# SamvitJ/Accel

Measured on AMD Instinct MI355X. Metric: frames/sec 1024x2048 Accel-18 kf=5, higher is better.
Workload: dtype f32 (storage, accumulation and results; the launch geometries the tuner picks include the fp32 MFMA, Winograd F(2x2,3x3) and, for most layers, 'fp16x2': each fp32 operand as TWO half terms hi + lo (22-23 significant bits, operands centred in the half range by exact powers of two: weights per channel

## Files before the change

### accel_amd/csrc/accel_hip.cpp

```cpp
#include <hip/hip_runtime.h>
#include <dlfcn.h>
#include <sys/stat.h>
#include <unistd.h>

#include <algorithm>
#include <cmath>
#include <cstdarg>
#include <cstdio>
#include <cstdlib>
#include <cstring>
#include <map>
#include <memory>
#include <sstream>
#include <string>
#include <vector>

#include "../../include/accel_hip.h"
#include "kernels.h"
#include "range.h"

static thread_local std::string g_err;

static int fail(int code, const char* fmt, ...)
{
// ... 479 lines not shown
        c.yH = op.b.H; c.yW = op.b.W;
        if (op.b.H > 2 * op.a.H || op.b.H < 2 * op.a.H - 1 || op.b.W > 2 * op.a.W || op.b.W < 2 * op.a.W - 1)
            return fail(ACCEL_ERR_PLAN, "deconv2x %s: output must be 2x the input (or one row / column less)", op.name.c_str());
    } else {
        int wkh = kh, wkw = kw;
        if (cols) kv_pair(kv, "wk", wkh, wkw, 3, 3);
        if (w->shape[0] != cout || w->shape[1] != cin || w->shape[2] != wkh || w->shape[3] != wkw)
            return fail(ACCEL_ERR_PARAM, "shape inconsistent for %s: need (%d,%d,%d,%d) got (%ld,%ld,%ld,%ld)",
                        wname.c_str(), cout, cin, wkh, wkw, (long)w->shape[0], (long)w->shape[1], (long)w->shape[2], (long)w->shape[3]);
        const int Kreal = wkh * wkw * cin_pad;
        c.K_pad = roundup(Kreal, 32);
        pack_conv_w(*w, cin_pad, rows, c.K_pad, packed);
        if (cols) { c.kh = c.kw = 1; c.Cin = Kreal; }
        else { c.kh = kh; c.kw = kw; c.Cin = cin_pad; }
        c.sh = sh; c.sw = sw; c.ph = ph; c.pw = pw; c.dh = dh; c.dw = dw;
        c.Ho = op.b.H; c.Wo = op.b.W;
        c.yH = op.b.H; c.yW = op.b.W;
        const int eh = (op.a.H + 2 * c.ph - c.dh * (c.kh - 1) - 1) / c.sh + 1;
        const int ew = (op.a.W + 2 * c.pw - c.dw * (c.kw - 1) - 1) / c.sw + 1;
        if (eh != op.b.H || ew != op.b.W)
            return fail(ACCEL_ERR_PLAN, "conv %s: output %dx%d does not match geometry %dx%d", op.name.c_str(), op.b.H, op.b.W, eh, ew);
        if (c.Cin > op.a.Cs) return fail(ACCEL_ERR_PLAN, "conv %s: input view narrower than Cin", op.name.c_str());
    }
    packed.resize(packed.size() + 256, 0.f);
    const char* env_dt = getenv("ACCEL_CONV_DTYPE");
    const int dflt = (p->f16 == 2 || (env_dt && !strcmp(env_dt, "bf16x3"))) ? 2 : (p->f16 || (env_dt && !strcmp(env_dt, "f16"))) ? 1 : 0;
    const int want_f16 = (int)kv_int(kv, "f16", dflt);
    c.f16 = (want_f16 && c.Cin % (want_f16 == 2 ? 4 : 8) == 0 && cout_store > 4) ? want_f16 : 0;
    void* dw_ = nullptr;
    if (c.f16 == 2) {
        std::vector<uint16_t> pb;
        pack_bf16x3(packed, c.deconv2x ? 4 : 1, rows, c.K_pad, pb, c.w_plane);
        if ((rc = dev_upload(p, pb.data(), pb.size() * sizeof(uint16_t), &dw_))) return rc;
    } else if (c.f16) {
        std::vector<_Float16> ph(packed.size());
        for (size_t i = 0; i < packed.size(); ++i) ph[i] = (_Float16)packed[i];
        if ((rc = dev_upload(p, ph.data(), ph.size() * sizeof(_Float16), &dw_))) return rc;
        if (!withheld("b3r")) {
            const int classes = c.deconv2x ? 4 : 1, steps = c.K_pad / 32;
            c.w_plane = (size_t)classes * rows * c.K_pad + 2 * (size_t)rows * 32;
            std::vector<_Float16> pr(c.w_plane, (_Float16)0.f);
            for (int cl = 0; cl < classes; ++cl)
                for (int n = 0; n < rows; ++n)
                    for (int k = 0; k < c.K_pad; ++k)
                        pr[((((size_t)cl * steps + k / 32) * 2 + ((k >> 4) & 1)) * rows + n) * 16 + (k & 15)] = ph[((size_t)cl * rows + n) * c.K_pad + k];
            void* d4 = nullptr;
            if ((rc = dev_upload(p, pr.data(), pr.size() * sizeof(_Float16), &d4))) return rc;
            c.wb3r = d4;
        }
    } else if ((rc = dev_upload(p, packed.data(), packed.size() * sizeof(float), &dw_))) return rc;
    c.w = static_cast<const float*>(dw_);
    {
        const int ft = (int)kv_int(kv, "tile", -1);
        const bool forced = (ft >= CONV_TILE_B3 && ft < CONV_TILE_B3D + CONV_TILE_B3D_N) || (ft >= 90 && ft <= 96);
        if (!c.f16 && c.Cin % 4 == 0 && cout_store > 4 && (!withheld("split") || forced)) {
            std::vector<uint16_t> pb;
            pack_bf16x3(packed, c.deconv2x ? 4 : 1, rows, c.K_pad, pb, c.w_plane);
            void* d3 = nullptr;
            if ((rc = dev_upload(p, pb.data(), pb.size() * sizeof(uint16_t), &d3))) return rc;
            c.wb3 = d3;
            const bool forced_r = (ft >= CONV_TILE_B3R && ft < CONV_TILE_B3D + CONV_TILE_B3D_N) || (ft >= 90 && ft <= 96);
            if (!withheld("b3r") || forced_r) {
                pack_bf16x3r(packed, c.deconv2x ? 4 : 1, rows, c.K_pad, pb, c.w_plane);
                void* d4 = nullptr;
                if ((rc = dev_upload(p, pb.data(), pb.size() * sizeof(uint16_t), &d4))) return rc;
                c.wb3r = d4;
            }
        } else if (forced && !(c.f16 == 1 && c.wb3r && ft >= CONV_TILE_B3R && ft < CONV_TILE_B3D + CONV_TILE_B3D_N)) {
            return fail(ACCEL_ERR_ARG, "conv %s: the bf16x3 kernel takes layers with more than "
                                       "4 output channels only", op.name.c_str());
        }
    }

    std::vector<float> scale(rows, 0.f), shift(rows, 0.f);
    for (int i = 0; i < cout; ++i) scale[i] = 1.f;
    if (kv_has(kv, "bn")) {
        std::vector<float> s, b;
        if ((rc = bn_fold(m, kv_str(kv, "bn"), (float)kv_f(kv, "eps", 1e-5), (int)kv_int(kv, "fixg", 0), cout, s, b))) return rc;
        for (int i = 0; i < cout; ++i) { scale[i] = s[i]; shift[i] = b[i]; }
    }
    if (kv_has(kv, "bias")) {
        const HostParam* bias = get_param(m, kv_str(kv, "bias"));
        if (!bias) return fail(ACCEL_ERR_PARAM, "%s not initialized", kv_str(kv, "bias").c_str());
        if ((int)bias->numel() != cout) return fail(ACCEL_ERR_PARAM, "shape inconsistent for %s", kv_str(kv, "bias").c_str());
        for (int i = 0; i < cout; ++i) shift[i] += bias->data[i] * scale[i];
    }
    if (kv_has(kv, "mul")) {
        const float mul = (float)kv_f(kv, "mul", 1.0);
        for (int i = 0; i < cout; ++i) { scale[i] *= mul; shift[i] *= mul; }
    }
    void *ds = nullptr, *db = nullptr;
    if ((rc = dev_upload(p, scale.data(), rows * sizeof(float), &ds)) ||
        (rc = dev_upload(p, shift.data(), rows * sizeof(float), &db))) return rc;
    c.scale = static_cast<const float*>(ds);
    c.shift = static_cast<const float*>(db);
    {
        const char* sp = getenv("ACCEL_SPLIT");
        const bool h2 = sp ? !strcmp(sp, "h2") : p->split == 1;
        if (c.wb3r && !c.f16 && h2) {
            std::vector<uint16_t> ph;
            std::vector<int> q;
            pack_h2r(packed, c.deconv2x ? 4 : 1, rows, c.K_pad, ph, c.w_plane, q);
            void *dh = nullptr, *dsh = nullptr;
            if ((rc = dev_upload(p, ph.data(), ph.size() * sizeof(uint16_t), &dh))) return rc;
            std::vector<float> sh(rows);
            for (int i = 0; i < rows; ++i) sh[i] = std::ldexp(scale[i], -q[i]);
            if ((rc = dev_upload(p, sh.data(), rows * sizeof(float), &dsh))) return rc;
            c.wh2r = dh;
            c.scale_h2 = static_cast<const float*>(dsh);
            ++p->n_h2;
        }
    }
    if (op.c.set) {
        std::vector<float> s2(rows, 0.f), b2(rows, 0.f), s, b;
// ... 413 lines not shown
    const ConvParams& c = op.conv;
    hipError_t e = hipSuccess;
    if (op.measure) e = launch_range_amax(c.x, (long)op.a.N * c.H * c.W, c.Cin, c.xCs, const_cast<unsigned*>(c.xr_slot), p->m->ctx->stream);
    if (e == hipSuccess && (op.measure || op.fold)) e = launch_range_fold(const_cast<unsigned*>(c.xr_slot), p->range_flag_dev, (int)(&op - p->ops.data()), p->m->ctx->stream);
    if (e != hipSuccess) return fail(ACCEL_ERR_HIP, "range pass of conv %s failed: %s", op.name.c_str(), hipGetErrorString(e));
    return 0;
}

static int run_eager(accel_plan* p)
{
    if (p->n_slots && launch_range_clear(p->range, p->n_slots, p->m->ctx->stream) != hipSuccess)
        return fail(ACCEL_ERR_HIP, "clearing the range slots of plan '%s' failed", p->role.c_str());
    for (size_t i = 0; i < p->ops.size(); ++i) {
        Op& op = p->ops[i];
        int rc = (op.measure || op.fold) ? launch_measure(p, op) : 0;
        if (!rc) rc = launch_op(p, op);
        if (rc) return rc;
        static const char* chk = getenv("ACCEL_CHECK_FINITE");
        if (chk && chk[0] == '1' && !p->gexec && (op.kind == OP_CONV || op.kind == OP_POOL || op.kind == OP_PREP_RGB) && p->n_slots) {
            const BufRef& o = op.b;
            if (o.esize == 4 && o.ptr && p->check_scratch) {
                unsigned* scratch = p->check_scratch;
                hipStream_t st = p->m->ctx->stream;
                launch_range_clear(scratch, 1, st);
                launch_range_amax(o.ptr, (long)o.N * o.H * o.W, roundup(o.C, 4), o.Cs, scratch, st);
                launch_range_fold(scratch, nullptr, 0, st);
                unsigned bits = 0;
                hipStreamSynchronize(st);
                hipMemcpy(&bits, scratch, 4, hipMemcpyDeviceToHost);
                if (bits >= 0x7F800000u) fprintf(stderr, "[accel check] plan %s op %zu %s %s: output holds a non-finite value (largest |x| bits 0x%08x)\n", p->role.c_str(), i, op.kind_name.c_str(), op.name.c_str(), bits);
            }
        }
    }
    return 0;
}

static int range_check(accel_plan* p)
{
    if (!p->range_flag || !*p->range_flag) return 0;
    const unsigned w = *p->range_flag, i = (w & 0x7FFFFFFFu) - 1u;
    *p->range_flag = 0u;
    return fail(ACCEL_ERR_RANGE, "plan '%s': the input of conv %s was not finite in an earlier run (the largest |value| stored into it was %s; fp16x2 "
                "form of the fp32 layers: the frames of that run are not trustworthy; ACCEL_SPLIT=b3 selects the bf16x3 form, which propagates "
                "non-finite values like fp32 arithmetic)",
                p->role.c_str(), i < p->ops.size() ? p->ops[i].name.c_str() : "?", (w & 0x80000000u) ? "a NaN" : "an infinity");
}

static bool conv_has_h2_form(const ConvParams& c) { return c.wh2r || c.wubh || c.wstemh; }
static bool conv_runs_h2(const ConvParams& c)
{
    if (c.f16 || c.narrow) return false;
    const int t = c.force_tile;
    return ((t == CONV_TILE_WINO_B3 || t == CONV_TILE_WINO_B3U || t == CONV_TILE_WINO_B3S) && c.wubh) || (t == CONV_TILE_STEM_B3 && c.wstemh) ||
           (((t >= CONV_TILE_B3R && t < CONV_TILE_B3R + 6) || (t >= 90 && t <= 96)) && c.wh2r);
}

static int assign_range_slots(accel_plan* p)
{
    std::map<int, int>& slot_of = p->slot_of;
    int n = 0;
    p->in_slot.assign(p->ops.size(), -1);
    for (size_t i = 0; i < p->ops.size(); ++i) {
        Op& op = p->ops[i];
        if (op.kind != OP_CONV || !conv_has_h2_form(op.conv)) continue;
        if (op.rs_in < 0) p->in_slot[i] = n++;
        else {
            auto it = slot_of.find(op.rs_in);
            if (it == slot_of.end()) it = slot_of.insert({op.rs_in, n++}).first;
            p->in_slot[i] = it->second;
        }
    }
    p->n_slots = n;
    if (!n) return 0;
    HIP_TRY(hipMalloc((void**)&p->range, (size_t)(n + 1) * RANGE_WORDS * sizeof(unsigned)));
    p->owned.push_back(p->range);
    HIP_TRY(hipMemset(p->range, 0, (size_t)(n + 1) * RANGE_WORDS * sizeof(unsigned)));
    p->check_scratch = p->range + (size_t)n * RANGE_WORDS;
    HIP_TRY(hipHostMalloc((void**)&p->range_flag, 2 * sizeof(unsigned), hipHostMallocMapped));
    p->range_flag[0] = p->range_flag[1] = 0u;
    HIP_TRY(hipHostGetDevicePointer((void**)&p->range_flag_dev, p->range_flag, 0));
    for (size_t i = 0; i < p->ops.size(); ++i)
        if (p->in_slot[i] >= 0) p->ops[i].conv.xr_slot = p->range + (size_t)p->in_slot[i] * RANGE_WORDS;
    return 0;
}

static void resolve_range_flags(accel_plan* p, bool (*counts)(const ConvParams&))
{
    const int n = p->n_slots;
    if (!n) return;
    std::vector<char> used(n, 0);
    for (size_t i = 0; i < p->ops.size(); ++i)
        if (p->in_slot[i] >= 0 && counts(p->ops[i].conv)) used[p->in_slot[i]] = 1;
    auto addr = [&](int id) -> unsigned* {
        auto it = id < 0 ? p->slot_of.end() : p->slot_of.find(id);
        return (it == p->slot_of.end() || !used[it->second]) ? nullptr : p->range + (size_t)it->second * RANGE_WORDS;
    };
    std::vector<int> state(n, 0);
    std::vector<char> dirty(n, 0);
    auto wrote = [&](int id, bool has_epilogue) {
        auto it = id < 0 ? p->slot_of.end() : p->slot_of.find(id);
        if (it == p->slot_of.end()) return;
        int& st = state[it->second];
        st = (has_epilogue && st != 2) ? 1 : 2;
        dirty[it->second] = 1;
    };
    for (size_t i = 0; i < p->ops.size(); ++i) {
        Op& op = p->ops[i];
// ... 128 lines not shown
    const char* e = getenv("ACCEL_AUTOTUNE");
    if (e && e[0] == '0') return 0;
    hipStream_t st = p->m->ctx->stream;
    tune_cache_load();
    bool tuned_any = false;
    struct Cand { int tile, split_target, no_split; };
    std::vector<std::vector<Cand>> cands(p->ops.size());
    size_t ws_need = p->ws_bytes;
    for (size_t i = 0; i < p->ops.size(); ++i) {
        Op& op = p->ops[i];
        if (op.kind != OP_CONV || op.conv.force_tile >= 0 || op.conv.narrow) continue;
        ConvParams c = op.conv;
        std::vector<Cand>& cs = cands[i];
        if (c.x_half || c.y_half || c.res_half) {
            for (int t : {CONV_TILE_B3D, CONV_TILE_B3D + 1, CONV_TILE_B3D + 2, CONV_TILE_B3D + 3, CONV_TILE_B3D + 6, CONV_TILE_B3D + 7}) {
                if ((t == CONV_TILE_B3D || t == CONV_TILE_B3D + 1) && c.Cout_store <= 128) continue;
                if ((t != CONV_TILE_B3D + 6) && c.Cout_store <= 64) continue;
                cs.push_back({t, 0, 0});
                ConvParams q = c;
                const size_t base = conv_apply(q, t, 0, 0);
                const int ks0 = q.ksplit;
                if (conv_apply(q, t, 1024, 0) && q.ksplit != ks0) cs.push_back({t, 1024, 0});
                if (base) cs.push_back({t, 0, 1});
            }
        }
        else if (c.f16 && c.Cout_store <= 32) { cs.push_back({3, 0, 0}); cs.push_back({3, 1024, 0}); }
        else if (c.Cout_store <= 32) {
            cs.push_back({4, 0, 0}); cs.push_back({4, 1024, 0}); cs.push_back({9, 0, 0}); cs.push_back({9, 1024, 0}); cs.push_back({3, 0, 0});
            if (c.wh2r && conv_halo_eligible(c) && !withheld("halo")) cs.push_back({CONV_TILE_HALO, 0, 1});
        }
        else {
            if (c.wu && !c.f16) {
                cs.push_back({CONV_TILE_WINO, 0, 0});
                ConvParams q = c;
                const size_t base = conv_apply(q, CONV_TILE_WINO, 0, 0);
                const int ks0 = q.ksplit;
                if (conv_apply(q, CONV_TILE_WINO, 1024, 0) && q.ksplit != ks0) cs.push_back({CONV_TILE_WINO, 1024, 0});
                if (base) cs.push_back({CONV_TILE_WINO, 0, 1});
            }
            if (c.wub && !c.f16) {
                for (int wt : {CONV_TILE_WINO_B3, CONV_TILE_WINO_B3U, CONV_TILE_WINO_B3S}) {
                    cs.push_back({wt, 0, 0});
                    ConvParams q = c;
                    const size_t base = conv_apply(q, wt, 0, 0);
                    const int ks0 = q.ksplit;
                    if (conv_apply(q, wt, 1024, 0) && q.ksplit != ks0) cs.push_back({wt, 1024, 0});
                    if (base) cs.push_back({wt, 0, 1});
                }
            }
            if (c.wstem && !c.f16) cs.push_back({CONV_TILE_STEM, 0, 0});
            if (c.wstemb && !c.f16) cs.push_back({CONV_TILE_STEM_B3, 0, 0});
            if (c.wws && !c.f16) cs.push_back({CONV_TILE_WS, 0, 0});
            if (c.wh2r && !c.f16 && conv_halo_eligible(c) && !withheld("halo")) cs.push_back({CONV_TILE_HALO, 0, 1});
            const int nb3 = c.wb3 ? 5 : 0;
            static const int tiles[] = {0, 1, 2, 3, 5, 6, 7, 8, 10, 11, 12, 13, 31, 32, 33, 34, 35,
                                        CONV_TILE_B3, CONV_TILE_B3 + 1, CONV_TILE_B3 + 2, CONV_TILE_B3 + 3, CONV_TILE_B3 + 4, CONV_TILE_B3 + 5,
                                        CONV_TILE_B3R, CONV_TILE_B3R + 1, CONV_TILE_B3R + 3, CONV_TILE_B3R + 4, CONV_TILE_B3R + 5};
            const bool no_deep = withheld("deep");
            for (int t : tiles) {
                if (t >= CONV_TILE_B3 && t < CONV_TILE_B3R && !nb3) continue;
                if (t >= CONV_TILE_B3R && !c.wb3r) continue;
                if (no_deep && t >= 31 && t <= 35) continue;
                if (c.K_pad % conv_tile_bk(t)) continue;
                if (c.f16 && !(t <= 3 || t == 10 || (c.f16 == 1 && t >= CONV_TILE_B3R && c.wb3r))) continue;
                cs.push_back({t, 0, 0});
                ConvParams q = c;
                const size_t base = conv_apply(q, t, 0, 0);
                const int ks0 = q.ksplit;
                if (conv_apply(q, t, 1024, 0) && q.ksplit != ks0) cs.push_back({t, 1024, 0});
                if (base) cs.push_back({t, 0, 1});
            }
        }
        if (const char* fw = getenv("ACCEL_WB3_FORCE"); fw && c.wub && !c.f16) {
            cs.clear();
            conv_apply(op.conv, atoi(fw), 0, 0);
            ConvParams q = op.conv;
            const size_t w = conv_plan_split(q);
            if (w > ws_need) ws_need = w;
            continue;
        }
        for (const Cand& k : cs) { ConvParams q = c; size_t w = conv_apply(q, k.tile, k.split_target, k.no_split); if (w > ws_need) ws_need = w; }
    }
    if (ws_need > p->ws_bytes) {
        float* nw = nullptr;
        HIP_TRY(hipMalloc((void**)&nw, ws_need));
        poison(nw, ws_need);
        p->owned.push_back(nw);
        p->ws = nw; p->ws_bytes = ws_need;
        for (Op& op : p->ops) if (op.kind == OP_CONV) op.conv.ws = p->ws;
    }
    struct TuneScratch {
        hipEvent_t e0 = nullptr, e1 = nullptr;
        void* scrub = nullptr;
        hipStream_t st;
        ~TuneScratch()
        {
            if (e0) hipEventDestroy(e0);
            if (e1) hipEventDestroy(e1);
            if (scrub) { hipStreamSynchronize(st); hipFree(scrub); }
        }
    } ts;
    ts.st = st;
    HIP_TRY(hipEventCreate(&ts.e0)); HIP_TRY(hipEventCreate(&ts.e1));
    hipEvent_t e0 = ts.e0, e1 = ts.e1;
    int rc = 0;
    const size_t scrub_bytes = (size_t)320 << 20;
// ... 1531 lines not shown
```

### accel_amd/csrc/conv_igemm.hip

```cpp
#include <hip/hip_runtime.h>
#include <cstdlib>
#include "kernels.h"
#include "conv_common.h"

#ifdef ACCEL_CONV_TIMELINE
__device__ unsigned long long g_conv_timeline[8 * 16384];
#define CONV_TL(slot) do { if (threadIdx.x == 0 && blockIdx.y == 0 && blockIdx.z == 0 && blockIdx.x < 16384) \
        g_conv_timeline[blockIdx.x * 8 + (slot)] = __builtin_amdgcn_s_memrealtime(); } while (0)
extern "C" int accel_debug_conv_timeline(unsigned long long* out, int n)
{
    return (int)hipMemcpyFromSymbol(out, HIP_SYMBOL(g_conv_timeline), sizeof(unsigned long long) * (size_t)n);
}
#else
#define CONV_TL(slot) do { } while (0)
#endif

#include "conv_epilogue.h"

template <int BM, int BN, int WGM, int WGN, int BK, int MID, int ABL = 0, int FAST = 0>
__global__ __launch_bounds__(64 * WGM * WGN) void conv_igemm_f32_kernel(ConvParams p)
{
    constexpr int LDK = BK + 4;
    constexpr int NTHR = 64 * WGM * WGN;
    constexpr int CPR = BK / 4;
// ... 935 lines not shown
    ConvParams p = p0;
    p.MT = (p.M + BM - 1) / BM;
    p.NT = (p.Cout_store + BN - 1) / BN;
    constexpr bool WDMA = WGM * WGN == 8;
    constexpr size_t lds = WDMA ? (size_t)(3 * BM * 40 + 2 * 3 * BN * 32) * sizeof(unsigned short) : (size_t)3 * (BM + BN) * 40 * sizeof(unsigned short);
    if (hipError_t e = ensure_dynamic_lds(reinterpret_cast<const void*>(&conv_igemm_b3_kernel<BM, BN, WGM, WGN, WDMA, true>), lds); e != hipSuccess) return e;
    if (hipError_t e = ensure_dynamic_lds(reinterpret_cast<const void*>(&conv_igemm_b3_kernel<BM, BN, WGM, WGN, WDMA, false>), lds); e != hipSuccess) return e;
    dim3 grid(p.MT * p.NT, p.deconv2x ? 4 : 1, p.ksplit > 1 ? p.ksplit : 1);
    if (p.Cin % 32 == 0) hipLaunchKernelGGL((conv_igemm_b3_kernel<BM, BN, WGM, WGN, WDMA, true>), grid, dim3(64 * WGM * WGN), lds, st, p, p.w_plane);
    else hipLaunchKernelGGL((conv_igemm_b3_kernel<BM, BN, WGM, WGN, WDMA, false>), grid, dim3(64 * WGM * WGN), lds, st, p, p.w_plane);
    hipError_t e = hipGetLastError();
    if (e != hipSuccess || p.ksplit <= 1) return e;
    const long total = (long)grid.y * p.M * (p.Cout_store / 4);
    hipLaunchKernelGGL(splitk_reduce_kernel, dim3((unsigned)((total + 255) / 256)), dim3(256), 0, st, p, (int)grid.y);
    return hipGetLastError();
}

int conv_pick_tile(const ConvParams& p)
{
    if (p.force_tile >= 0) return p.force_tile;
    if (p.x_half || p.y_half || p.res_half) return p.Cout_store <= 64 ? CONV_TILE_B3D + 6 : CONV_TILE_B3D + 2;
    const long classes = p.deconv2x ? 4 : 1;
    const int cs = p.Cout_store;
    if (cs <= 32) return p.f16 ? 3 : 4;
    auto blocks = [&](int bm, int bn) {
        return classes * ((p.M + bm - 1) / bm) * (long)((cs + bn - 1) / bn);
    };
    if (cs <= 64) return blocks(128, 64) >= 512 ? 1 : 3;
    if (blocks(128, 128) < 64) return 3;
    if (cs % 128 == 0 || cs > 256) {
        if (blocks(128, 128) >= 512) return 0;
        if (blocks(128, 64) >= 512) return 1;
        if (blocks(64, 128) >= 384) return 2;
        return 3;
    }
    if (blocks(128, 64) >= 512) return 1;
    return 3;
}

hipError_t launch_splitk_reduce(const ConvParams& p, int classes, hipStream_t st)
{
    const long total = (long)classes * p.M * (p.Cout_store / 4);
    hipLaunchKernelGGL(splitk_reduce_kernel, dim3((unsigned)((total + 255) / 256)), dim3(256), 0, st, p, classes);
    return hipGetLastError();
}

int conv_tile_bk(int tile) { return tile == 13 ? 64 : tile == 15 ? 16 : 32; }

bool conv_tile_valid(int tile)
{
#ifdef ACCEL_CONV_DIAG
    if ((tile >= 20 && tile <= 30) || (tile >= 90 && tile <= 96)) return true;
#endif
    return (tile >= 0 && tile <= 19) || (tile >= 31 && tile <= 35) || tile == CONV_TILE_WINO || tile == CONV_TILE_WINO_B3 || tile == CONV_TILE_WINO_B3U || tile == CONV_TILE_WINO_B3S || tile == CONV_TILE_STEM || tile == CONV_TILE_STEM_B3 || tile == CONV_TILE_WS || tile == CONV_TILE_HALO ||
           (tile >= CONV_TILE_B3 && tile < CONV_TILE_B3 + 8) || (tile >= CONV_TILE_B3R + 3 && tile <= CONV_TILE_B3R + 5) ||
           (tile >= CONV_TILE_B3D && tile < CONV_TILE_B3D + CONV_TILE_B3D_N);
}

static void tile_dims(int tile, int& bm, int& bn)
{
    static const int BMs[20] = {128, 128, 64, 64, 128, 128, 128, 64, 64, 128, 128, 128, 64, 64, 256, 128, 128, 64, 128, 64};
    static const int BNs[20] = {128, 64, 128, 64, 32, 128, 64, 128, 64, 32, 128, 64, 128, 64, 128, 128, 128, 64, 128, 64};
    if (tile == CONV_TILE_B3 + 5) { bm = 256; bn = 128; return; }
    if (tile == CONV_TILE_B3R || (tile >= 90 && tile <= 96)) { bm = 128; bn = 128; return; }
    if (tile == CONV_TILE_B3R + 1) { bm = 128; bn = 64; return; }
    if (tile == CONV_TILE_B3R + 3 || tile == CONV_TILE_B3R + 4) { bm = 128; bn = 256; return; }
    if (tile == CONV_TILE_B3R + 5) { bm = 128; bn = 128; return; }
    if (tile == CONV_TILE_B3D || tile == CONV_TILE_B3D + 4) { bm = 256; bn = 256; return; }
    if (tile == CONV_TILE_B3D + 1 || tile == CONV_TILE_B3D + 5) { bm = 128; bn = 256; return; }
    if (tile == CONV_TILE_B3D + 2 || tile == CONV_TILE_B3D + 3) { bm = 128; bn = 128; return; }
    if (tile == CONV_TILE_B3D + 6) { bm = 128; bn = 64; return; }
    if (tile == CONV_TILE_B3D + 7) { bm = 256; bn = 128; return; }
    if (tile >= CONV_TILE_B3 && tile < CONV_TILE_B3 + 5) { static const int g[5] = {0, 1, 2, 3, 10}; tile = g[tile - CONV_TILE_B3]; }
    if (tile >= 31 && tile <= 35) { static const int g[5] = {3, 0, 2, 1, 4}; tile = g[tile - 31]; }
    if (tile >= 20) tile = (tile == 23 || (tile >= 26 && tile != 29)) ? 3 : 0;
    if (tile < 0 || tile > 19) tile = 3;
    bm = BMs[tile]; bn = BNs[tile];
}

size_t conv_plan_split(ConvParams& p)
{
    p.ksplit = 1; p.kt_per_split = 0;
    if (p.no_split || p.narrow) return 0;
    int bm, bn;
    const int tile = conv_pick_tile(p);
    if (tile == CONV_TILE_STEM || tile == CONV_TILE_STEM_B3 || tile == CONV_TILE_WS || tile == CONV_TILE_HALO) return 0;
    if (tile == CONV_TILE_WINO) {
        const long blocks = ((p.M / 4 + 63) / 64) * (long)conv_wino_rows(p.Cout_store) / 64;
        const int KT = p.Cin / 8, min_steps = 4;
        const int min_blocks = p.split_target > 0 ? p.split_target : 256;
        const int target = p.split_target > 0 ? p.split_target : 512;
        if (blocks >= min_blocks || KT < 2 * min_steps) return 0;
        int want = (int)((target + blocks - 1) / blocks);
        int ks = want < KT / min_steps ? want : KT / min_steps;
        if (ks < 2) return 0;
        p.kt_per_split = ((KT + ks - 1) / ks + 1) / 2 * 2;
        p.ksplit = (KT + p.kt_per_split - 1) / p.kt_per_split;
        if (p.ksplit < 2) { p.ksplit = 1; p.kt_per_split = 0; return 0; }
        return (size_t)p.ksplit * p.M * p.Cout_store * sizeof(float);
    }
    if (tile == CONV_TILE_WINO_B3 || tile == CONV_TILE_WINO_B3U || tile == CONV_TILE_WINO_B3S) {
        const long blocks = (tile == CONV_TILE_WINO_B3U ? conv_wino_b3u_blocks(p, nullptr) : tile == CONV_TILE_WINO_B3S ? conv_wino_b3s_blocks(p, nullptr) : (long)((p.M / 4 + 63) / 64)) * (long)conv_wino_rows(p.Cout_store) / 64;
        const int KT = p.Cin / 16, min_steps = 4;
        const int min_blocks = p.split_target > 0 ? p.split_target : 256;
        const int target = p.split_target > 0 ? p.split_target : 512;
        if (blocks >= min_blocks || KT < 2 * min_steps) return 0;
        int want = (int)((target + blocks - 1) / blocks);
        int ks = want < KT / min_steps ? want : KT / min_steps;
        if (ks < 2) return 0;
        p.kt_per_split = (KT + ks - 1) / ks;
        p.ksplit = (KT + p.kt_per_split - 1) / p.kt_per_split;
        if (p.ksplit < 2) { p.ksplit = 1; p.kt_per_split = 0; return 0; }
        return (size_t)p.ksplit * p.M * p.Cout_store * sizeof(float);
    }
    tile_dims(tile, bm, bn);
    const long classes = p.deconv2x ? 4 : 1;
    const long blocks = classes * ((p.M + bm - 1) / bm) * ((p.Cout_store + bn - 1) / bn);
    const int KT = p.K_pad / conv_tile_bk(tile);
    const int min_blocks = p.split_target > 0 ? p.split_target : 256;
    const int target = p.split_target > 0 ? p.split_target : 768;
    const int min_steps = 4;
    if (blocks >= min_blocks || KT < 2 * min_steps) return 0;
    int want = (int)((target + blocks - 1) / blocks);
    int ks = want < KT / min_steps ? want : KT / min_steps;
    if (ks < 2) return 0;
    p.kt_per_split = (KT + ks - 1) / ks;
    if (tile >= CONV_TILE_B3D && tile < CONV_TILE_B3D + CONV_TILE_B3D_N && p.f16 == 1) p.kt_per_split = (p.kt_per_split + 1) / 2 * 2;
    p.ksplit = (KT + p.kt_per_split - 1) / p.kt_per_split;
    if (p.ksplit < 2) { p.ksplit = 1; p.kt_per_split = 0; return 0; }
    return (size_t)p.ksplit * classes * p.M * p.Cout_store * sizeof(float);
}

hipError_t launch_conv_igemm(const ConvParams& p, hipStream_t st)
{
    if (p.narrow) return launch_conv_narrow(p, st);
    if (p.force_tile == CONV_TILE_WINO) return launch_conv_wino(p, st);
    if (p.force_tile == CONV_TILE_WINO_B3 || p.force_tile == CONV_TILE_WINO_B3U || p.force_tile == CONV_TILE_WINO_B3S) {
        ConvParams q = p;
        if (p.wubh && !p.f16) {
            q.wub = p.wubh;
            q.wub_bytes = p.wub_bytes / 3 * 2;
            q.scale = p.scale_h2w;
            q.xr = p.xr_slot;
            q.f16 = 3;
        }
        if (p.force_tile == CONV_TILE_WINO_B3S) return launch_conv_wino_b3s(q, st);
        return launch_conv_wino_b3(q, st, p.force_tile == CONV_TILE_WINO_B3U);
    }
    if (p.force_tile == CONV_TILE_STEM) return launch_conv_stem(p, st);
    if (p.force_tile == CONV_TILE_STEM_B3) {
        if (p.wstemh && !p.f16) {
            ConvParams q = p;
            q.wstemb = p.wstemh;
            q.scale = p.scale_h2s;
            q.xr = p.xr_slot;
            q.f16 = 3;
            return launch_conv_stem_b3(q, st);
        }
        return launch_conv_stem_b3(p, st);
    }
    if (p.force_tile == CONV_TILE_WS) return launch_conv_ws(p, st);
    if (p.force_tile == CONV_TILE_HALO) {
        if (p.f16 || !p.wh2r || p.x_half || p.y_half || p.res_half) return hipErrorInvalidValue;
        ConvParams q = p;
        q.w = static_cast<const float*>(p.wh2r);
        q.w_bytes = p.w_bytes / 2;
        q.scale = p.scale_h2;
        q.xr = p.xr_slot;
        q.f16 = 3;
        return launch_conv_halo(q, st);
    }
    const int b3d_tile = (p.force_tile < 0 && (p.x_half || p.y_half || p.res_half)) ? conv_pick_tile(p) : p.force_tile;
    if (b3d_tile >= CONV_TILE_B3D && b3d_tile < CONV_TILE_B3D + CONV_TILE_B3D_N) {
        if (!p.wb3r || p.f16 != 1) return hipErrorInvalidValue;
        ConvParams q = p;
        q.w = static_cast<const float*>(p.wb3r);
        return launch_conv_b3d(q, b3d_tile, st);
    }
    if (p.x_half || p.y_half || p.res_half) return hipErrorInvalidValue;
    if (p.force_tile >= CONV_TILE_B3R && p.force_tile < CONV_TILE_B3R + 6 && p.f16 == 1) {
        if (!p.wb3r) return hipErrorInvalidValue;
        ConvParams q = p;
        q.w = static_cast<const float*>(p.wb3r);
        return launch_conv_b3r(q, p.force_tile, st);
    }
    if (((p.force_tile >= CONV_TILE_B3R && p.force_tile < CONV_TILE_B3R + 6) || (p.force_tile >= 90 && p.force_tile <= 96)) && !p.f16 && p.wh2r) {
        ConvParams q = p;
        q.w = static_cast<const float*>(p.wh2r);
        q.w_bytes = p.w_bytes / 2;
        q.scale = p.scale_h2;
        q.xr = p.xr_slot;
        q.f16 = 3;
        return launch_conv_b3r(q, p.force_tile, st);
    }
    if (((p.force_tile >= CONV_TILE_B3R && p.force_tile < CONV_TILE_B3R + 6) || (p.force_tile >= 90 && p.force_tile <= 96)) && !p.f16) {
        if (!p.wb3r) return hipErrorInvalidValue;
        ConvParams q = p;
        q.w = static_cast<const float*>(p.wb3r);
        q.w_bytes = p.w_bytes / 2;
        q.f16 = 2;
        return launch_conv_b3r(q, p.force_tile, st);
    }
    if (p.force_tile >= CONV_TILE_B3 && p.force_tile < CONV_TILE_B3 + 6 && !p.f16) {
        if (!p.wb3) return hipErrorInvalidValue;
        ConvParams q = p;
        q.w = static_cast<const float*>(p.wb3);
        q.w_bytes = p.w_bytes / 2;
        q.f16 = 2;
        switch (p.force_tile - CONV_TILE_B3) {
            case 0: return launch_b3<128, 128, 2, 2>(q, st);
            case 1: return launch_b3<128, 64, 2, 2>(q, st);
            case 2: return launch_b3<64, 128, 2, 2>(q, st);
            case 3: return launch_b3<64, 64, 2, 2>(q, st);
            case 5: return launch_b3<256, 128, 4, 2>(q, st);
            default: return launch_b3<128, 128, 2, 4>(q, st);
        }
    }
    if (p.f16 == 2) {
        switch (conv_pick_tile(p)) {
            case 0: case 5: return launch_b3<128, 128, 2, 2>(p, st);
            case 1: case 6: return launch_b3<128, 64, 2, 2>(p, st);
            case 2: case 7: return launch_b3<64, 128, 2, 2>(p, st);
            case 10: return launch_b3<128, 128, 2, 4>(p, st);
// ... 62 lines not shown
```

### accel_amd/csrc/kernels.h

```cpp
#pragma once
#include <vector>
#include <hip/hip_runtime.h>
#include <stddef.h>

struct ConvParams {
    const float* x;
    const float* w;
    float* y;
    float* y2;
    const float* res;
    const float* scale; const float* shift;
    const float* scale2; const float* shift2;
    int H, W;
    int Cin;
    int xCs;
    int Ho, Wo;
    int kh, kw, sh, sw, ph, pw, dh, dw;
    int K_pad;
    int Cout_store;
    int Cout;
    int yCs, y2Cs, resCs;
    int M;
    int act;
    float slope;
// ... 25 lines not shown
    unsigned wws_bytes;
    const void* wb3r;
    const void* wub;
    unsigned wub_bytes;
    const void* wh2r;
    const float* scale_h2;
    const void* wstemh;
    const float* scale_h2s;
    const void* wubh;
    const float* scale_h2w;
    const unsigned* xr;
    const unsigned* xr_slot;
    unsigned* yr;
    unsigned* y2r;
    int x_half, y_half, res_half;
};

hipError_t launch_conv_igemm(const ConvParams& p, hipStream_t st);
int conv_pick_tile(const ConvParams& p);
int conv_tile_bk(int tile);
bool conv_tile_valid(int tile);
#define CONV_TILE_WINO 40
#define CONV_TILE_WINO_B3S 43
#define CONV_TILE_WINO_B3U 42
#define CONV_TILE_WINO_B3 41
bool conv_wino_eligible(const ConvParams& p);
int conv_wino_rows(int cout_store);
void conv_wino_pack(const float* w, int Cout, int Cin, int cin_pad, int rows, float* out);
hipError_t launch_conv_wino(const ConvParams& p, hipStream_t st);
bool conv_wino_b3_eligible(const ConvParams& p);
void conv_wino_b3_pack(const float* w, int Cout, int Cin, int rows, std::vector<unsigned short>& out);
void conv_wino_b3_pack_h2(const float* w, int Cout, int Cin, int rows, std::vector<unsigned short>& out, std::vector<int>& qexp);
hipError_t launch_conv_wino_b3(const ConvParams& p, hipStream_t st, bool union_loader = false);
long conv_wino_b3u_blocks(const ConvParams& p, int* bhs);
long conv_wino_b3s_blocks(const ConvParams& p, int* bhs);
hipError_t launch_conv_wino_b3s(const ConvParams& p, hipStream_t st);
hipError_t launch_splitk_reduce(const ConvParams& p, int classes, hipStream_t st);
#define CONV_TILE_STEM 50
#define CONV_TILE_STEM_B3 51
bool conv_stem_b3_eligible(const ConvParams& p);
void conv_stem_b3_pack(const float* w, int Cout, std::vector<unsigned short>& out);
void conv_stem_b3_pack_h2(const float* w, int Cout, std::vector<unsigned short>& out, std::vector<int>& qexp);
hipError_t launch_conv_stem_b3(const ConvParams& p, hipStream_t st);
bool conv_stem_eligible(const ConvParams& p);
void conv_stem_pack(const float* w, int Cout, float* out);
int conv_stem_pack_floats();
hipError_t launch_conv_stem(const ConvParams& p, hipStream_t st);
#define CONV_TILE_HALO 78
bool conv_halo_eligible(const ConvParams& p);
hipError_t launch_conv_halo(const ConvParams& p, hipStream_t st);
#define CONV_TILE_B3 70
#define CONV_TILE_B3R 76
hipError_t launch_conv_b3r(const ConvParams& p, int tile, hipStream_t st);
#define CONV_TILE_B3D 82
#define CONV_TILE_B3D_N 8
bool conv_b3d_eligible(const ConvParams& p);
hipError_t launch_conv_b3d(const ConvParams& p, int tile, hipStream_t st);
#define CONV_TILE_WS 60
bool conv_ws_eligible(const ConvParams& p);
size_t conv_ws_pack_floats(int Cin, int cout_store);
void conv_ws_pack(const float* w, int Cout, int Cin, int cout_store, float* out);
hipError_t launch_conv_ws(const ConvParams& p, hipStream_t st);
size_t conv_plan_split(ConvParams& p);

hipError_t launch_prep_rgb(const float* src, float* dst, int H, int W,
                           const float* scale3, const float* shift3, int N, hipStream_t st, const float* const* slot = nullptr, unsigned* yr = nullptr);
hipError_t launch_prep_flow(const float* cur, const float* prev, float* dst, int H, int W,
                            int N, hipStream_t st, const float* const* cur_slot = nullptr, const float* const* prev_slot = nullptr, unsigned* yr = nullptr);
hipError_t launch_set_slot(const void** slot, const void* value, hipStream_t st);
hipError_t launch_frames_u8(const unsigned char* src, int n, int h, int w, size_t pitch, const double* means_bgr, int out_h, int out_w, double step,
                            int H, int W, float* dst, hipStream_t st);
hipError_t launch_labels_source(const unsigned char* labels, int n, int H, int W, int out_h, int out_w, int h, int w, unsigned char* dst, size_t dst_pitch,
                                hipStream_t st);
hipError_t launch_labels_hist(const unsigned char* labels, int n, int H, int W, int out_h, int out_w, const unsigned char* gt, int h, int w, size_t gt_pitch,
                              int ncls, unsigned long long* hist, hipStream_t st);
hipError_t launch_labels_colour(const unsigned char* labels, int n, int H, int W, int out_h, int out_w, int h, int w, const unsigned char* palette_rgb,
                                int rgb_order, const unsigned char* frame, size_t frame_pitch, int alpha, unsigned char* dst, size_t dst_pitch, hipStream_t st);
hipError_t launch_confidence(const float* scores, int n, int ncls, int H, int W, int out_h, int out_w, int h, int w, int is_prob, unsigned char* conf,
                             size_t conf_pitch, float* margin, size_t margin_pitch, unsigned char* second, size_t second_pitch, unsigned long long* hist,
                             hipStream_t st);

struct PoolParams {
    const float* x; float* y;
    int C4;
    int xCs, yCs;
    int H, W, Ho, Wo;
    int kh, kw, sh, sw, ph, pw;
    int is_max;
    const float* scale; const float* shift;
    int relu;
    int N;
    size_t x_img, y_img;
    unsigned* yr;
};
hipError_t launch_pool(const PoolParams& p, hipStream_t st);

hipError_t launch_flow_warp(const float* feat, int fCs, const float* flow, int flCs,
                            float* out, int oCs, int C, int H, int W,
                            float* out2, int o2Cs, const float* bias, int N, hipStream_t st, unsigned* yr = nullptr, unsigned* y2r = nullptr);

struct DcnColsParams {
    const float* x; const float* off; float* col;
    int C, xCs, offCs, colCs;
    int H, W, Ho, Wo;
    int kh, kw, sh, sw, ph, pw, dh, dw;
    int dg;
// ... 33 lines not shown
```

Before: 620.4.

## Add A-stationary fp16x2 1x1 conv kernel as autotuner candidate

Adds a new 1x1 stride-1 convolution kernel that loads a 64-row activation tile once into LDS, splitting each value into hi/lo half planes, and then sweeps all output-channel chunks of 256 against it. Weights stream from global memory with double-buffered loads, and three MFMAs per step give the fp16x2 product. The kernel is registered as a tuner candidate for eligible layers, so it only runs when it wins. The aim is to avoid re-reading and re-splitting activations for every output-channel tile. In exchange it uses large LDS per block, which may cut occupancy, and it serialises the channel chunks within each block.

After: 620.5, median of 3. About the same (+0.0%).

```diff
diff --git a/accel_amd/csrc/accel_hip.cpp b/accel_amd/csrc/accel_hip.cpp
--- a/accel_amd/csrc/accel_hip.cpp
+++ b/accel_amd/csrc/accel_hip.cpp
@@ -555,14 +555,14 @@
     c.w = static_cast<const float*>(dw_);
     {
         const int ft = (int)kv_int(kv, "tile", -1);
-        const bool forced = (ft >= CONV_TILE_B3 && ft < CONV_TILE_B3D + CONV_TILE_B3D_N) || (ft >= 90 && ft <= 96);
+        const bool forced = (ft >= CONV_TILE_B3 && ft < CONV_TILE_B3D + CONV_TILE_B3D_N) || (ft >= 90 && ft <= 96) || ft == CONV_TILE_AS1X1;
         if (!c.f16 && c.Cin % 4 == 0 && cout_store > 4 && (!withheld("split") || forced)) {
             std::vector<uint16_t> pb;
             pack_bf16x3(packed, c.deconv2x ? 4 : 1, rows, c.K_pad, pb, c.w_plane);
             void* d3 = nullptr;
             if ((rc = dev_upload(p, pb.data(), pb.size() * sizeof(uint16_t), &d3))) return rc;
             c.wb3 = d3;
-            const bool forced_r = (ft >= CONV_TILE_B3R && ft < CONV_TILE_B3D + CONV_TILE_B3D_N) || (ft >= 90 && ft <= 96);
+            const bool forced_r = (ft >= CONV_TILE_B3R && ft < CONV_TILE_B3D + CONV_TILE_B3D_N) || (ft >= 90 && ft <= 96) || ft == CONV_TILE_AS1X1;
             if (!withheld("b3r") || forced_r) {
                 pack_bf16x3r(packed, c.deconv2x ? 4 : 1, rows, c.K_pad, pb, c.w_plane);
                 void* d4 = nullptr;
@@ -1082,7 +1082,7 @@
     if (c.f16 || c.narrow) return false;
     const int t = c.force_tile;
     return ((t == CONV_TILE_WINO_B3 || t == CONV_TILE_WINO_B3U || t == CONV_TILE_WINO_B3S) && c.wubh) || (t == CONV_TILE_STEM_B3 && c.wstemh) ||
-           (((t >= CONV_TILE_B3R && t < CONV_TILE_B3R + 6) || (t >= 90 && t <= 96)) && c.wh2r);
+           (((t >= CONV_TILE_B3R && t < CONV_TILE_B3R + 6) || (t >= 90 && t <= 96) || t == CONV_TILE_AS1X1) && c.wh2r);
 }
 
 static int assign_range_slots(accel_plan* p)
@@ -1317,6 +1317,7 @@
             if (c.wstemb && !c.f16) cs.push_back({CONV_TILE_STEM_B3, 0, 0});
             if (c.wws && !c.f16) cs.push_back({CONV_TILE_WS, 0, 0});
             if (c.wh2r && !c.f16 && conv_halo_eligible(c) && !withheld("halo")) cs.push_back({CONV_TILE_HALO, 0, 1});
+            if (c.wh2r && !c.f16 && conv_as1x1_eligible(c) && !withheld("as1x1")) cs.push_back({CONV_TILE_AS1X1, 0, 1});
             const int nb3 = c.wb3 ? 5 : 0;
             static const int tiles[] = {0, 1, 2, 3, 5, 6, 7, 8, 10, 11, 12, 13, 31, 32, 33, 34, 35,
                                         CONV_TILE_B3, CONV_TILE_B3 + 1, CONV_TILE_B3 + 2, CONV_TILE_B3 + 3, CONV_TILE_B3 + 4, CONV_TILE_B3 + 5,
diff --git a/accel_amd/csrc/conv_as1x1.hip b/accel_amd/csrc/conv_as1x1.hip
--- /dev/null
+++ b/accel_amd/csrc/conv_as1x1.hip
@@ -0,0 +1,132 @@
+#include <hip/hip_runtime.h>
+#include "kernels.h"
+#include "conv_common.h"
+#include "conv_epilogue.h"
+
+typedef _Float16 f16x8a __attribute__((ext_vector_type(8)));
+
+#define AS1X1_BM 64
+#define AS1X1_MAX_CIN 512
+
+static size_t as1x1_lds(int Cin) { return (size_t)2 * AS1X1_BM * (Cin + 8) * sizeof(unsigned short); }
+
+template <int BM>
+__global__ __launch_bounds__(512, 4) void conv_as1x1_kernel(ConvParams p, size_t wplane, int rowsB)
+{
+    constexpr int NTHR = 512, MI = BM / 32;
+    constexpr int UPP = 4;
+    extern __shared__ __attribute__((aligned(16))) unsigned short smem_as[];
+    const int tid = threadIdx.x, lane = tid & 63, wave = __builtin_amdgcn_readfirstlane(tid >> 6);
+    const int m0 = blockIdx.x * BM;
+    const int LDK = p.Cin + 8;
+    const RangeScale rs = range_prologue(p.xr);
+    const float xs = rs.s;
+
+    {
+        const __amdgpu_buffer_rsrc_t xr = make_rsrc(p.x, p.x_bytes);
+        const int cpr = p.Cin >> 3, nunits = BM * cpr;
+        const float inv_cpr = 1.0f / (float)cpr;
+        for (int base = 0; base < nunits; base += NTHR * UPP) {
+            f32x4 lo[UPP], hi[UPP];
+            int sidx[UPP];
+#pragma unroll
+            for (int i = 0; i < UPP; ++i) {
+                const int u = base + tid + NTHR * i;
+                int row, cu;
+                divmod_small(u, cpr, inv_cpr, row, cu);
+                const bool ok = u < nunits && m0 + row < p.M;
+                const unsigned off = ok ? (unsigned)(((m0 + row) * p.xCs + cu * 8) * 4) : OOB;
+                lo[i] = buf_load4(xr, off);
+                hi[i] = buf_load4(xr, ok ? off + 16u : OOB);
+                sidx[i] = u < nunits ? row * LDK + cu * 8 : -1;
+            }
+#pragma unroll
+            for (int i = 0; i < UPP; ++i) {
+                f16x8a h, l;
+#pragma unroll
+                for (int e = 0; e < 8; ++e) {
+                    const float v = e < 4 ? lo[i][e] : hi[i][e - 4];
+                    h[e] = (_Float16)(v * xs);
+                    l[e] = (_Float16)__builtin_fmaf(v, xs, -(float)h[e]);
+                }
+                if (sidx[i] >= 0) {
+                    *reinterpret_cast<i32x4*>(smem_as + sidx[i]) = __builtin_bit_cast(i32x4, h);
+                    *reinterpret_cast<i32x4*>(smem_as + BM * LDK + sidx[i]) = __builtin_bit_cast(i32x4, l);
+                }
+            }
+        }
+    }
+    __syncthreads();
+
+    const int ncw = p.Cout_store > 32 * wave ? (p.Cout_store - 32 * wave + 255) >> 8 : 0;
+    if (ncw == 0) return;
+    const int frow = lane & 31, half = lane >> 5;
+    const int nhs = p.Cin >> 4;
+    const unsigned short* wbase = reinterpret_cast<const unsigned short*>(p.w);
+    const __amdgpu_buffer_rsrc_t wall = make_rsrc(wbase, (unsigned)(2 * wplane) + (unsigned)((size_t)rowsB * p.K_pad * 2) + (unsigned)(rowsB * 128));
+    const unsigned hstep = (unsigned)rowsB * 32u, plane_b = (unsigned)(2 * wplane);
+    const unsigned voff0 = (unsigned)((32 * wave + frow) * 32 + half * 16);
+    i32x4 bcur[2], bnext[2];
+    auto load_b = [&](i32x4 (&b)[2], int chunk, int hs) {
+        const unsigned voff = voff0 + (unsigned)chunk * (256u * 32u);
+#pragma unroll
+        for (int pl = 0; pl < 2; ++pl) b[pl] = __builtin_amdgcn_raw_buffer_load_b128(wall, voff, (unsigned)pl * plane_b + (unsigned)hs * hstep, 0);
+    };
+
+    f32x16 acc[MI][1];
+#pragma unroll
+    for (int i = 0; i < MI; ++i)
+#pragma unroll
+        for (int e = 0; e < 16; ++e) acc[i][0][e] = 0.f;
+
+    const unsigned short* arow = smem_as + frow * LDK + half * 8;
+    const int HoWo = p.Ho * p.Wo;
+    load_b(bcur, 0, 0);
+    for (int chunk = 0; chunk < ncw; ++chunk) {
+        for (int hs = 0; hs < nhs; ++hs) {
+            const bool last = hs + 1 == nhs;
+            load_b(bnext, last ? (chunk + 1 < ncw ? chunk + 1 : 0) : chunk, last ? 0 : hs + 1);
+            i32x4 fa[MI][2];
+#pragma unroll
+            for (int pl = 0; pl < 2; ++pl)
+#pragma unroll
+                for (int i = 0; i < MI; ++i) fa[i][pl] = *reinterpret_cast<const i32x4*>(arow + (pl * BM + i * 32) * LDK + hs * 16);
+            const f16x8a b0 = __builtin_bit_cast(f16x8a, bcur[0]), b1 = __builtin_bit_cast(f16x8a, bcur[1]);
+#pragma unroll
+            for (int i = 0; i < MI; ++i) {
+                const f16x8a a0 = __builtin_bit_cast(f16x8a, fa[i][0]), a1 = __builtin_bit_cast(f16x8a, fa[i][1]);
+                f32x16 c = acc[i][0];
+                c = __builtin_amdgcn_mfma_f32_32x32x16_f16(a1, b0, c, 0, 0, 0);
+                c = __builtin_amdgcn_mfma_f32_32x32x16_f16(a0, b1, c, 0, 0, 0);
+                acc[i][0] = __builtin_amdgcn_mfma_f32_32x32x16_f16(a0, b0, c, 0, 0, 0);
+            }
+            bcur[0] = bnext[0]; bcur[1] = bnext[1];
+        }
+        int m0c = m0;
+        asm volatile("" : "+s"(m0c));
+        conv_epilogue<MI, 1, 8>(p, acc, m0c, chunk * 256, 0, wave, lane, 0, 0, HoWo, rs.inv);
+#pragma unroll
+        for (int i = 0; i < MI; ++i)
+#pragma unroll
+            for (int e = 0; e < 16; ++e) acc[i][0][e] = 0.f;
+    }
+}
+
+bool conv_as1x1_eligible(const ConvParams& p)
+{
+    return p.kh == 1 && p.kw == 1 && p.sh == 1 && p.sw == 1 && p.ph == 0 && p.pw == 0 && p.dh == 1 && p.dw == 1 && !p.deconv2x && !p.narrow &&
+           p.Cin % 32 == 0 && p.Cin <= AS1X1_MAX_CIN && p.K_pad == p.Cin && p.Ho == p.H && p.Wo == p.W && !p.x_half && !p.y_half && !p.res_half;
+}
+
+hipError_t launch_conv_as1x1(const ConvParams& p0, hipStream_t st)
+{
+    ConvParams p = p0;
+    if (!conv_as1x1_eligible(p) || p.f16 != 3 || p.ksplit > 1) return hipErrorInvalidValue;
+    p.MT = (p.M + AS1X1_BM - 1) / AS1X1_BM;
+    p.NT = 1;
+    const size_t lds = as1x1_lds(p.Cin);
+    if (hipError_t e = ensure_dynamic_lds(reinterpret_cast<const void*>(&conv_as1x1_kernel<AS1X1_BM>), as1x1_lds(AS1X1_MAX_CIN)); e != hipSuccess) return e;
+    const int rowsB = (int)(p.w_bytes / ((unsigned)p.K_pad * 2u));
+    hipLaunchKernelGGL(conv_as1x1_kernel<AS1X1_BM>, dim3(p.MT), dim3(512), lds, st, p, p.w_plane, rowsB);
+    return hipGetLastError();
+}
diff --git a/accel_amd/csrc/conv_igemm.hip b/accel_amd/csrc/conv_igemm.hip
--- a/accel_amd/csrc/conv_igemm.hip
+++ b/accel_amd/csrc/conv_igemm.hip
@@ -1011,7 +1011,7 @@
 #ifdef ACCEL_CONV_DIAG
     if ((tile >= 20 && tile <= 30) || (tile >= 90 && tile <= 96)) return true;
 #endif
-    return (tile >= 0 && tile <= 19) || (tile >= 31 && tile <= 35) || tile == CONV_TILE_WINO || tile == CONV_TILE_WINO_B3 || tile == CONV_TILE_WINO_B3U || tile == CONV_TILE_WINO_B3S || tile == CONV_TILE_STEM || tile == CONV_TILE_STEM_B3 || tile == CONV_TILE_WS || tile == CONV_TILE_HALO ||
+    return (tile >= 0 && tile <= 19) || (tile >= 31 && tile <= 35) || tile == CONV_TILE_WINO || tile == CONV_TILE_WINO_B3 || tile == CONV_TILE_WINO_B3U || tile == CONV_TILE_WINO_B3S || tile == CONV_TILE_STEM || tile == CONV_TILE_STEM_B3 || tile == CONV_TILE_WS || tile == CONV_TILE_HALO || tile == CONV_TILE_AS1X1 ||
            (tile >= CONV_TILE_B3 && tile < CONV_TILE_B3 + 8) || (tile >= CONV_TILE_B3R + 3 && tile <= CONV_TILE_B3R + 5) ||
            (tile >= CONV_TILE_B3D && tile < CONV_TILE_B3D + CONV_TILE_B3D_N);
 }
@@ -1025,6 +1025,7 @@
     if (tile == CONV_TILE_B3R + 1) { bm = 128; bn = 64; return; }
     if (tile == CONV_TILE_B3R + 3 || tile == CONV_TILE_B3R + 4) { bm = 128; bn = 256; return; }
     if (tile == CONV_TILE_B3R + 5) { bm = 128; bn = 128; return; }
+    if (tile == CONV_TILE_AS1X1) { bm = 64; bn = 256; return; }
     if (tile == CONV_TILE_B3D || tile == CONV_TILE_B3D + 4) { bm = 256; bn = 256; return; }
     if (tile == CONV_TILE_B3D + 1 || tile == CONV_TILE_B3D + 5) { bm = 128; bn = 256; return; }
     if (tile == CONV_TILE_B3D + 2 || tile == CONV_TILE_B3D + 3) { bm = 128; bn = 128; return; }
@@ -1128,6 +1129,16 @@
         q.xr = p.xr_slot;
         q.f16 = 3;
         return launch_conv_halo(q, st);
+    }
+    if (p.force_tile == CONV_TILE_AS1X1) {
+        if (p.f16 || !p.wh2r || p.x_half || p.y_half || p.res_half) return hipErrorInvalidValue;
+        ConvParams q = p;
+        q.w = static_cast<const float*>(p.wh2r);
+        q.w_bytes = p.w_bytes / 2;
+        q.scale = p.scale_h2;
+        q.xr = p.xr_slot;
+        q.f16 = 3;
+        return launch_conv_as1x1(q, st);
     }
     const int b3d_tile = (p.force_tile < 0 && (p.x_half || p.y_half || p.res_half)) ? conv_pick_tile(p) : p.force_tile;
     if (b3d_tile >= CONV_TILE_B3D && b3d_tile < CONV_TILE_B3D + CONV_TILE_B3D_N) {
diff --git a/accel_amd/csrc/kernels.h b/accel_amd/csrc/kernels.h
--- a/accel_amd/csrc/kernels.h
+++ b/accel_amd/csrc/kernels.h
@@ -101,6 +101,9 @@
 #define CONV_TILE_B3 70
 #define CONV_TILE_B3R 76
 hipError_t launch_conv_b3r(const ConvParams& p, int tile, hipStream_t st);
+#define CONV_TILE_AS1X1 97
+bool conv_as1x1_eligible(const ConvParams& p);
+hipError_t launch_conv_as1x1(const ConvParams& p, hipStream_t st);
 #define CONV_TILE_B3D 82
 #define CONV_TILE_B3D_N 8
 bool conv_b3d_eligible(const ConvParams& p);
```
